# pierric/smart-chess-rust

Measured on AMD Instinct MI355X. Metric: MCTS simulations/sec (whole node), self-play rollout=180, at 1/2/4/8 MI355X, higher is better.
Workload: dtype bf16

## Files before the change

smart-chess-rust_amd/csrc/chess_history.hpp:

```cpp
#pragma once
#include "chess_rules.hpp"

namespace sc {

template <class Chain>
SC_HD bool is_repetition(const Chain& ch, int idx, int count) {
    bb_t key0 = ch.pos(idx).key;
    int i = idx;
    for (;;) {
        if (count <= 1) return true;
        if (i < count - 1) break;
        bool irrev = (ch.pos(i).flags & F_IRREV) != 0;
        i--;
        if (irrev) break;
        if (ch.pos(i).key == key0) count--;
    }
    return false;
}

enum { T_NONE = 0, T_CHECKMATE = 1, T_STALEMATE = 2, T_INSUFFICIENT = 3, T_SEVENTYFIVE = 4, T_FIVEFOLD = 5, T_FIFTY = 6, T_THREEFOLD = 7 };

template <class Chain>
SC_HD int outcome_claim_draw(const Chain& ch, int idx, int* winner) {
    const Position& p = ch.pos(idx);
    move_t buf1[MAX_MOVES], buf2[MAX_MOVES];
    MoveList l{buf1, 0};
    bool in_check = gen_legal(p, l);
    *winner = -1;
    if (in_check && l.n == 0) {
        *winner = !p.turn;
        return T_CHECKMATE;
    }
    if (insufficient_side(p, WHITE) && insufficient_side(p, BLACK)) return T_INSUFFICIENT;
    if (l.n == 0) return T_STALEMATE;
    if (p.halfmove >= 150) return T_SEVENTYFIVE;
    if (is_repetition(ch, idx, 5)) return T_FIVEFOLD;
    if (p.halfmove >= 100) return T_FIFTY;
    if (p.halfmove >= 99) {
        for (int i = 0; i < l.n; i++) {
            if (is_zeroing(p, l.m[i])) continue;
            Position q = p;
            make_move(q, l.m[i]);
            MoveList l2{buf2, 0};
            gen_legal(q, l2);
            if (q.halfmove >= 100 && l2.n > 0) return T_FIFTY;
        }
    }
    int lo = idx;
    while (lo > 0 && !(ch.pos(lo).flags & F_IRREV)) lo--;
    int cnt = 1;
    for (int i = lo; i < idx; i++)
        if (ch.pos(i).key == p.key) cnt++;
    if (cnt >= 3) return T_THREEFOLD;
    for (int j = 0; j < l.n; j++) {
        Position q = p;
        make_move(q, l.m[j]);
        int c2 = q.key == p.key ? 1 : 0;
        for (int i = lo; i < idx; i++)
            if (ch.pos(i).key == q.key) c2++;
        if (c2 >= 2) return T_THREEFOLD;
    }
    return T_NONE;
}

template <class Chain>
SC_HD void encode_cell(const Chain& ch, int idx, int px, int8_t* cell ) {
    int turn = ch.pos(idx).turn;
    int src = turn == BLACK ? (px ^ 56) : px;
    bb_t sb = bit(src);
    for (int j = 0; j < 8; j++) {
        int8_t* c = cell + 14 * j;
        for (int k = 0; k < 14; k++) c[k] = 0;
        if (j > idx) continue;
        const Position& h = ch.pos(idx - j);
        if ((h.occ[0] | h.occ[1]) & sb) {
            int t = piece_type_at(h, src);
            int is_white = (h.occ[WHITE] & sb) ? 1 : 0;
            int mover_side = turn == BLACK ? !is_white : is_white;
            c[t + (mover_side ? 0 : 6)] = 1;
        }
        c[12] = (h.flags & F_REP2) ? 1 : 0;
        c[13] = (h.flags & F_REP3) ? 1 : 0;
    }
}
SC_HD void encode_meta(const Position& p, int32_t* meta ) {
    int t = p.turn;
    uint8_t mk_ = t ? 1 : 4, mq = t ? 2 : 8, ok = t ? 4 : 1, oq = t ? 8 : 2;
    meta[0] = t;
    meta[1] = p.fullmove;
    meta[2] = (p.castling & mk_) != 0;
    meta[3] = (p.castling & mq) != 0;
    meta[4] = (p.castling & ok) != 0;
    meta[5] = (p.castling & oq) != 0;
    meta[6] = p.halfmove;
}

template <class Chain>
SC_HD uint8_t repetition_flags(const Chain& ch, int idx) {
    uint8_t f = 0;
    if (is_repetition(ch, idx, 2)) f |= F_REP2;
    if (is_repetition(ch, idx, 3)) f |= F_REP3;
    return f;
}

}
```

smart-chess-rust_amd/csrc/mcts_kernels.hip:

```cpp
#include "search_expand.hpp"

#include "launchers.hpp"

namespace sc {
__global__ __launch_bounds__(64) void k_debug_find_max(const float* u, int n, int* out) {
    const int lane = threadIdx.x;
    if (n <= 64) {
        const int r = wave_argmax_last_lane(lane < n ? u[lane] : 0.f, lane < n);
        if (lane == 0) out[0] = r;
    } else if (lane == 0) {
        out[0] = -2;
    }
    float best_u = 0.f;
    int best_i = -1;
#pragma unroll
    for (int r = 0; r < 4; r++) {
        const int i = lane + 64 * r;
        if (i < n) {
            const float v = u[i];
            if (best_i < 0 || v >= best_u) {
                best_u = v;
                best_i = i;
            }
        }
    }
    const int r4 = wave_argmax_last(best_u, best_i);
    if (lane == 0) out[1] = r4;
}

__global__ __launch_bounds__(64) void k_synth_eval(SpParams p) {
    const int g = blockIdx.x, lane = threadIdx.x;
    GameCtl& c = p.ctl[g];
    if (c.status != ST_ACTIVE || c.leaf_kind != LK_EVAL) return;
    const Position& pos = p.tpos[(size_t)g * p.tpos_cap + c.n_exp];
    uint64_t h = synth_pos_hash(pos) ^ p.synth_salt;
    int n = c.n_legal;
    const uint16_t* lm = p.legal_mv + (size_t)g * MAXC;
    if (p.evaluator == SYNTH_UNIFORM) {
        for (int i = lane; i < n; i += 64) p.prior[(size_t)g * MAXC + i] = 1.0f / (float)n;
        if (lane == 0) p.value[g] = 0.0f;
        return;
    }
    const bool coarse = p.evaluator == SYNTH_COARSE;
    unsigned long long sum = 0;
    for (int i = lane; i < n; i += 64) sum += coarse ? 1u + (synth_weight(h, lm[i]) >> 22) : synth_weight(h, lm[i]);
    sum = scw::wave_sum_u64(sum);
    float fs = (float)sum;
    for (int i = lane; i < n; i += 64)
        p.prior[(size_t)g * MAXC + i] = (float)(coarse ? 1u + (synth_weight(h, lm[i]) >> 22) : synth_weight(h, lm[i])) / fs;
    if (lane == 0) {
        const float v = synth_value(h);
        p.value[g] = coarse ? (v < -0.5f ? -0.5f : v >= 0.5f ? 0.5f : 0.0f) : v;
    }
}

__device__ inline int match_white(const SpParams& p, unsigned long long k) { return p.match_colours ? (int)(k & 1) : 0; }
__device__ inline unsigned long long match_ordinal(SpParams& p, int lane, int side) {
    const unsigned long long total = (unsigned long long)p.total_games;
    if (!p.match_colours && side) return total;
    unsigned long long n = 0;
    if (lane == 0) n = atomicAdd(&p.cnt->match_next[side], 1ULL);
    n = __shfl(n, 0, 64);
    const unsigned long long k = p.match_colours ? 2ULL * n + (unsigned long long)side : n;
    return k < total ? k : total;
}
__device__ inline int match_line_of(const SpParams& p, const MatchLines& ln, unsigned long long k) {
    return (int)((p.match_colours ? k >> 1 : k) % (unsigned long long)ln.n);
}
__device__ inline void match_copy_line(SpParams& p, int g, int lane, const Position* line, int len) {
    constexpr int W = (int)(sizeof(Position) / 8);
    static_assert(sizeof(Position) % 8 == 0, "a record is copied in 8-byte words");
    const unsigned long long* src = reinterpret_cast<const unsigned long long*>(line);
    unsigned long long* hist = reinterpret_cast<unsigned long long*>(p.hist + (size_t)g * p.hist_cap);
    unsigned long long* root = reinterpret_cast<unsigned long long*>(p.tpos + (size_t)g * p.tpos_cap);
    const int words = (len + 1) * W;
    wave_sync();
    for (int i = lane; i < words; i += 64) hist[i] = src[i];
    if (lane < W) root[lane] = src[len * W + lane];
    if (lane == 0) {
        p.ctl[g].ply = len;
        p.ctl[g].start_ply = len;
    }
}
__device__ inline void match_slot_start(SpParams& p, const MatchLines& ln, int g, int lane) {
    GameCtl& c = p.ctl[g];
    const int st = c.status, side = p.match_side & 1;
    const unsigned long long total = (unsigned long long)p.total_games;
    unsigned long long k;
    if (st == ST_MATCH_WAIT) {
        k = c.game_id - p.first_game_id;
    } else if (st == ST_IDLE) {
        k = match_ordinal(p, lane, side);
        if (k >= total) k = match_ordinal(p, lane, side ^ 1);
        if (k >= total) return;
    } else {
        return;
    }
    wave_sync();
    int len = 0;
    const Position* line = nullptr;
    if (ln.n > 0) {
        const int i = match_line_of(p, ln, k);
        const uint32_t a = ln.off[i], b = ln.off[i + 1];
        line = ln.tab + a;
        len = (int)(b - a) - 1;
    }
    if (side == (match_white(p, k) ^ (len & 1))) {
        try_start_game(p, g, lane, k);
        int now = 0;
        if (lane == 0) {
            now = c.status;
            if (now == ST_PENDING) c.status = ST_MATCH_WAIT;
        }
        if (len > 0 && __shfl(now, 0, 64) == ST_ACTIVE) match_copy_line(p, g, lane, line, len);
    } else if (lane == 0) {
        c.status = ST_MATCH_WAIT;
        c.leaf_kind = LK_NONE;
        c.game_id = p.first_game_id + k;
    }
}
__global__ __launch_bounds__(64) void k_match_boundary(SpParams p, MatchLines ln, int phase) {
    const int g = blockIdx.x, lane = threadIdx.x;
    if (phase == 1) {
        match_slot_start(p, ln, g, lane);
        return;
    }
    GameCtl& c = p.ctl[g];
    if (lane != 0 || c.status != ST_IDLE || c.trace_slot < 0) return;
    const TraceHdr& th = p.thdr[c.trace_slot];
    const int w = match_white(p, c.game_id - p.first_game_id);
    const int r = !th.has_outcome ? 3 : th.winner == 1 ? 0 : th.winner == 0 ? 1 : 2;
    p.match_tally()[((size_t)g * 2 + w) * 4 + r] += 1;
    c.trace_slot = -1;
}

__global__ __launch_bounds__(64) void k_init_slots(SpParams p, MatchLines ln) {
    const int g = blockIdx.x, lane = threadIdx.x;
    uint4* b = reinterpret_cast<uint4*>(p.boards + (size_t)g * 7168);
    for (int i = lane; i < 448; i += 64) b[i] = make_uint4(0, 0, 0, 0);
    if (lane < 8) p.meta[(size_t)g * 8 + lane] = 0;
    if (lane == 0) p.n_legal[g] = 0;
    if (p.match_recycle) {
        if (lane == 0) {
            p.ctl[g].status = ST_IDLE;
            p.ctl[g].leaf_kind = LK_NONE;
            p.ctl[g].trace_slot = -1;
        }
        wave_sync();
        match_slot_start(p, ln, g, lane);
        return;
    }
    if (g == 0 && lane == 0)
        atomicAdd(&p.cnt->next_game, (unsigned long long)(p.n_slots < p.total_games ? p.n_slots : p.total_games));
    if (g >= p.total_games) {
        if (lane == 0) {
            p.ctl[g].status = ST_IDLE;
            p.ctl[g].leaf_kind = LK_NONE;
        }
        return;
    }
    try_start_game(p, g, lane, (unsigned long long)g);
}

__global__ __launch_bounds__(64) void k_debug_choose_child(int n_cases, const int32_t* n_act, const int32_t* nc, const float* temperature,
                                                           const float* u, int tie_random, const float* w, const int32_t* w_off, int w_max,
                                                           int32_t* choice, float* total) {
    const int c = blockIdx.x, lane = threadIdx.x;
    if (c >= n_cases) return;
    float tot;
    const int ch = choose_child(n_act + (size_t)c * MAXC, uniform(nc[c]), temperature[c], u[c], tie_random, lane, w + uniform(w_off[c]), w_max, &tot);
    if (lane == 0) {
        choice[c] = ch;
        total[c] = tot;
    }
}

__global__ __launch_bounds__(64) void k_mcts(SpParams p, int do_expand, int do_select) {
    const int g = blockIdx.x, lane = threadIdx.x;
    __shared__ __attribute__((aligned(16))) int8_t s_stage[7168];
    __shared__ move_t s_moves[MAXC];
    __shared__ Position s_pos;
    __shared__ Position s_hist[8];
    __shared__ uint16_t s_ps[DEPTH_LDS];
    constexpr bool SC_ST = true;
    SC_STAMP(0);
    GameCtl cs_pre{};
    bool cs_pre_valid = false;
    if (do_expand) {
        dev_expand(p, g, lane, &s_pos, cs_pre, cs_pre_valid);
        __builtin_amdgcn_wave_barrier();
    }
    SC_STAMP(1);
    if (do_select) dev_select(p, g, lane, s_stage, s_moves, &s_pos, s_ps, s_hist, cs_pre, cs_pre_valid);
}

__global__ __launch_bounds__(64) void k_match_tally(const int32_t* tally, int n_slots, long long* out) {
    const int j = threadIdx.x;
    if (j >= 8) return;
    long long s = 0;
    for (int g = 0; g < n_slots; g++) s += tally[(size_t)g * 8 + j];
    out[j] = s;
}

__global__ __launch_bounds__(64) void k_open_lines(int n_lines, const uint16_t* moves, const uint32_t* move_off, Position* tab,
                                                   const uint32_t* rec_off, int32_t* status, Bases bases) {
    const int i = blockIdx.x, lane = threadIdx.x;
    if (i >= n_lines) return;
    __shared__ move_t s_moves[MAXC];
    __shared__ Position s_np;
    const uint16_t* mv = moves + move_off[i];
    const int nm = (int)(move_off[i + 1] - move_off[i]);
    const int pad = (int)(rec_off[i + 1] - rec_off[i]) - 1 - nm;
    Position* hist = tab + rec_off[i] + (pad > 0 ? pad : 0);
    Position cur = chain_start(bases, i, true);
    if (lane == 0) {
        Position none;
        set_startpos(none);
#pragma unroll
        for (int t = 0; t < 6; t++) none.pcs[t] = 0;
        none.occ[0] = none.occ[1] = 0;
        none.castling = 0;
        for (int k = 0; k < pad; k++) tab[rec_off[i] + k] = none;
        hist[0] = cur;
    }
    __syncthreads();
    int st = 0;
    for (int j = 0; j < nm; j++) {
        int nlm = 0;
        gen_legal_wave(cur, s_moves, lane, nlm);
        __syncthreads();
        bool found = false;
        for (int k = 0; k < nlm; k++)
            if (s_moves[k] == mv[j]) found = true;
        __syncthreads();
        if (!found) {
            st = -(j + 1);
            break;
        }
        replay_step(cur, mv[j], j, hist, hist, &s_np, lane);
    }
    if (st == 0) {
        int n = 0, winner = -1;
        gen_legal_wave(cur, s_moves, lane, n);
        __syncthreads();
        const HistChain hc{hist};
        if (outcome_claim_draw(hc, nm, &winner) != T_NONE || n == 0) st = 1;
    }
    if (lane == 0 && pad > 0) hist[0].flags = F_IRREV;
    if (lane == 0) status[i] = st;
}

__global__ __launch_bounds__(64) void k_set_position(SpParams p, int g, const uint16_t* moves, int n_moves, const Position* base) {
    const int lane = threadIdx.x;
    GameCtl& c = p.ctl[g];
    Position* hist = p.hist + (size_t)g * p.hist_cap;
    Position* tpos = p.tpos + (size_t)g * p.tpos_cap;
    __shared__ Position s_np;
    Position cur;
    if (base) {
        cur = uniform(*base);
    } else {
        set_startpos(cur);
        cur.key = position_key(cur);
    }
    if (lane == 0) hist[0] = cur;
    __syncthreads();
    for (int i = 0; i < n_moves && i + 1 < p.hist_cap; i++) replay_step(cur, moves[i], i, hist, tpos, &s_np, lane);
    if (lane == 0) {
        const size_t nb = (size_t)g * p.node_cap;
        tpos[0] = cur;
        p.N[nb] = 0;
        p.W[nb] = 0.0f;
        p.H[nb] = NodeHdr{-1, 0, 0};
        c.ply = n_moves;
        c.start_ply = n_moves;
        c.sim = 0;
        c.n_nodes = 1;
        c.n_exp = 1;
        c.leaf_kind = LK_NONE;
        c.rollout_cur = p.rollout;
        c.status = ST_ACTIVE;
    }
}

}

namespace scl {
void init_slots(const sc::SpParams& p, const sc::MatchLines& lines, hipStream_t s) {
    hipLaunchKernelGGL(sc::k_init_slots, dim3(p.n_slots), dim3(64), 0, s, p, lines);
}
void mcts(const sc::SpParams& p, int do_expand, int do_select, hipStream_t s) {
    hipLaunchKernelGGL(sc::k_mcts, dim3(p.n_slots), dim3(64), 0, s, p, do_expand, do_select);
}
void synth_eval(const sc::SpParams& p, hipStream_t s) { hipLaunchKernelGGL(sc::k_synth_eval, dim3(p.n_slots), dim3(64), 0, s, p); }
void debug_find_max(const float* d_u, int n, int* d_out, hipStream_t s) { hipLaunchKernelGGL(sc::k_debug_find_max, dim3(1), dim3(64), 0, s, d_u, n, d_out); }
void debug_choose_child(int n_cases, const int32_t* d_n_act, const int32_t* d_nc, const float* d_temperature, const float* d_u, int tie_random,
                        const float* d_w, const int32_t* d_w_off, int w_max, int32_t* d_choice, float* d_total, hipStream_t s) {
    if (n_cases <= 0) return;
    hipLaunchKernelGGL(sc::k_debug_choose_child, dim3(n_cases), dim3(64), 0, s, n_cases, d_n_act, d_nc, d_temperature, d_u, tie_random,
                       d_w, d_w_off, w_max, d_choice, d_total);
}
void match_boundary(const sc::SpParams& p, const sc::MatchLines& lines, hipStream_t s) {
    hipLaunchKernelGGL(sc::k_match_boundary, dim3(p.n_slots), dim3(64), 0, s, p, lines, 0);
    hipLaunchKernelGGL(sc::k_match_boundary, dim3(p.n_slots), dim3(64), 0, s, p, lines, 1);
}
void open_lines(int n_lines, const uint16_t* d_moves, const uint32_t* d_move_off, sc::Position* d_tab, const uint32_t* d_rec_off,
                int32_t* d_status, const sc::Bases& bases, hipStream_t s) {
    if (n_lines <= 0) return;
    hipLaunchKernelGGL(sc::k_open_lines, dim3(n_lines), dim3(64), 0, s, n_lines, d_moves, d_move_off, d_tab, d_rec_off, d_status, bases);
}
void match_tally(const int32_t* d_tally, int n_slots, long long* d_out, hipStream_t s) {
    hipLaunchKernelGGL(sc::k_match_tally, dim3(1), dim3(64), 0, s, d_tally, n_slots, d_out);
}
void set_position(const sc::SpParams& p, int slot, const uint16_t* d_moves, int n_moves, hipStream_t s, const sc::Position* d_base) {
    hipLaunchKernelGGL(sc::k_set_position, dim3(1), dim3(64), 0, s, p, slot, d_moves, n_moves, d_base);
}
}
```

smart-chess-rust_amd/csrc/position_chain.hpp:

```cpp
#pragma once
#include <hip/hip_runtime.h>

#include "chess_history.hpp"
#include "chess_rules_wave.hpp"
#include "encode_types.hpp"
#include "wave_util.hpp"

namespace sc {

using scw::uniform, scw::wave_sync;
__device__ __forceinline__ Position uniform(const Position& q) {
    Position r;
#pragma unroll
    for (int t = 0; t < 6; t++) r.pcs[t] = uniform(q.pcs[t]);
    r.occ[0] = uniform(q.occ[0]);
    r.occ[1] = uniform(q.occ[1]);
    r.key = uniform(q.key);
    r.turn = (uint8_t)uniform((int)q.turn);
    r.castling = (uint8_t)uniform((int)q.castling);
    r.ep = (int8_t)uniform((int)q.ep);
    r.flags = (uint8_t)uniform((int)q.flags);
    r.halfmove = (uint16_t)uniform((int)q.halfmove);
    r.fullmove = (uint16_t)uniform((int)q.fullmove);
    return r;
}

__device__ __forceinline__ Position chain_start(const Bases& b, int g, bool keyed) {
    Position cur;
    const int bi = b.rec ? uniform(b.idx[g]) : -1;
    if (bi >= 0) {
        cur = uniform(b.rec[bi]);
    } else {
        set_startpos(cur);
        if (keyed) cur.key = position_key(cur);
    }
    if (!keyed) cur.key = cur.flags = 0;
    return cur;
}

struct DevChain {
    const Position* hist;
    int root_ply;
    const Position* tpos;
    const uint16_t* ps_by_depth;
    const Position* leaf;
    int leaf_idx;
    __device__ const Position& pos(int i) const {
        if (i <= root_ply) return hist[i];
        if (i == leaf_idx) return *leaf;
        return tpos[ps_by_depth[i - root_ply]];
    }
};
struct HistChain {
    const Position* hist;
    __device__ const Position& pos(int i) const { return hist[i]; }
};

template <class Chain>
__device__ inline uint8_t rep_flags_wave(const Chain& ch, int idx, bb_t key0, int lane) {
    int matches = 0;
    for (int base = 0;; base += 64) {
        int i = idx - base - lane;
        bool valid = i >= 1;
        bool irrev = false, match = false;
        if (valid) {
            irrev = (ch.pos(i).flags & F_IRREV) != 0;
            match = ch.pos(i - 1).key == key0;
        }
        unsigned long long stopmask = __ballot(irrev || !valid);
        unsigned long long matchmask = __ballot(match && valid);
        bool stopped = stopmask != 0;
        if (stopped) {
            int first = __ffsll((long long)stopmask) - 1;
            matchmask &= first == 0 ? 0ULL : (~0ULL >> (64 - first));
        }
        matches += __popcll(matchmask);
        if (stopped || matches >= 2) break;
    }
    return (uint8_t)((matches >= 1 ? F_REP2 : 0) | (matches >= 2 ? F_REP3 : 0));
}

template <class Chain>
__device__ inline void stage_history(const Chain& ch, int idx, int lane, Position* s_hist) {
    const int j = lane >> 3, w = lane & 7;
    if (j <= idx) {
        const unsigned long long* src = reinterpret_cast<const unsigned long long*>(&ch.pos(idx - j));
        unsigned long long* dst = reinterpret_cast<unsigned long long*>(&s_hist[j]);
        dst[w] = src[w];
        if (w < 2) dst[8 + w] = src[8 + w];
    }
}

__device__ inline void encode_wave(const Position* s_hist, int n_hist, int lane, int8_t* stage, int8_t* out, int32_t* meta_out) {
    uint4* cell16 = reinterpret_cast<uint4*>(stage + lane * 112);
#pragma unroll
    for (int k = 0; k < 7; k++) cell16[k] = make_uint4(0, 0, 0, 0);
    int8_t* cell = stage + lane * 112;
    const int turn = s_hist[0].turn;
    int src = turn == BLACK ? (lane ^ 56) : lane;
    bb_t sb = bit(src);
    for (int j = 0; j < n_hist; j++) {
        const Position& h = s_hist[j];
        bb_t ow = h.occ[WHITE], ob = h.occ[BLACK];
        if ((ow | ob) & sb) {
            int t = 0;
#pragma unroll
            for (int k = 1; k < 6; k++)
                if (h.pcs[k] & sb) t = k;
            int is_white = (ow & sb) ? 1 : 0;
            int mover_side = turn == BLACK ? !is_white : is_white;
            cell[14 * j + t + (mover_side ? 0 : 6)] = 1;
        }
        uint8_t f = h.flags;
        cell[14 * j + 12] = (f & F_REP2) ? 1 : 0;
        cell[14 * j + 13] = (f & F_REP3) ? 1 : 0;
    }
    if (out) {
        uint4* o16 = reinterpret_cast<uint4*>(out + lane * 112);
#pragma unroll
        for (int k = 0; k < 7; k++) o16[k] = cell16[k];
    }
    if (lane == 0) {
        int32_t m[7];
        encode_meta(s_hist[0], m);
#pragma unroll
        for (int k = 0; k < 7; k++) meta_out[k] = m[k];
        meta_out[7] = 0;
    }
}

__device__ __forceinline__ void write_meta_row(const RowOut& o, int g, int lane) {
    if (!o.meta || lane >= 7) return;
    const int32_t* m = o.meta_s + (size_t)g * 7;
    int32_t v = m[lane];
    if (o.apply_mirror) v = lane == 0 ? 1 - m[0] : lane == 1 ? m[1] + (m[0] == 1 ? 1 : 0) : lane == 2 ? m[4] : lane == 3 ? m[5] : lane == 4 ? m[2] : lane == 5 ? m[3] : v;
    if (o.layout == 1) static_cast<float*>(o.meta)[(size_t)g * 7 + lane] = (float)v;
    else static_cast<int32_t*>(o.meta)[(size_t)g * 7 + lane] = v;
}

__device__ inline bb_t position_key_wave(const Position& p, int lane, bool ep_legal) {
    bb_t h = 0;
    if ((all_occ(p) >> lane) & 1) h = psq_key(piece_type_at(p, lane), (int)((p.occ[WHITE] >> lane) & 1), lane);
    unsigned lo = (unsigned)h, hi = (unsigned)(h >> 32);
    for (int o = 32; o > 0; o >>= 1) {
        lo ^= (unsigned)__shfl_xor((int)lo, o, 64);
        hi ^= (unsigned)__shfl_xor((int)hi, o, 64);
    }
    return (((bb_t)hi << 32) | lo) ^ state_key(p.turn, p.castling, ep_legal ? p.ep : -1);
}

__device__ inline void replay_step(Position& cur, move_t m, int i, Position* hist, const Position* tpos, Position* s_np, int lane) {
    make_move(cur, m);
    if (lane == 0) *s_np = cur;
    __syncthreads();
    DevChain ch{hist, i, tpos, nullptr, s_np, i + 1};
    uint8_t rf = rep_flags_wave(ch, i + 1, cur.key, lane);
    cur.flags = (uint8_t)((cur.flags & F_IRREV) | rf);
    __syncthreads();
    if (lane == 0) hist[i + 1] = cur;
    __threadfence_block();
    __syncthreads();
}

}
```

smart-chess-rust_amd/csrc/rules_host_api.cpp:

```cpp
#include <stdlib.h>
#include <string.h>
#include <vector>

#include "chess_history.hpp"

using namespace sc;

struct sct_state {
    std::vector<Position> hist;
    std::vector<move_t> moves;
    const Position& pos(int i) const { return hist[(size_t)i]; }
};

static void finalize_rep(sct_state* s) {
    int idx = (int)s->hist.size() - 1;
    s->hist[(size_t)idx].flags |= repetition_flags(*s, idx);
}

extern "C" {

sct_state* sct_new() {
    sct_state* s = new sct_state();
    Position p;
    set_startpos(p);
    p.key = position_key(p);
    s->hist.push_back(p);
    return s;
}
void sct_free(sct_state* s) { delete s; }
void sct_reset(sct_state* s) {
    Position p;
    set_startpos(p);
    p.key = position_key(p);
    s->hist.assign(1, p);
    s->moves.clear();
}
int sct_set_fen(sct_state* s, const char* fen) {
    Position p;
    memset(&p, 0, sizeof p);
    int r = 7, f = 0;
    const char* c = fen;
    const char* names = "pnbrqk";
    for (; *c && *c != ' '; c++) {
        if (*c == '/') { r--; f = 0; continue; }
        if (*c >= '1' && *c <= '8') { f += *c - '0'; continue; }
        bool white = *c >= 'A' && *c <= 'Z';
        char lc = (char)(white ? *c + 32 : *c);
        const char* q = strchr(names, lc);
        if (!q || r < 0 || f > 7) return -1;
        int sq = r * 8 + f;
        p.pcs[q - names] |= bit(sq);
        p.occ[white ? WHITE : BLACK] |= bit(sq);
        f++;
    }
    if (*c != ' ') return -1;
    c++;
    p.turn = *c == 'w';
    c++;
    while (*c == ' ') c++;
    for (; *c && *c != ' '; c++) {
        if (*c == 'K') p.castling |= 1;
        if (*c == 'Q') p.castling |= 2;
        if (*c == 'k') p.castling |= 4;
        if (*c == 'q') p.castling |= 8;
    }
    bb_t wk = p.pcs[KING] & p.occ[WHITE], bk = p.pcs[KING] & p.occ[BLACK];
    bb_t wr = p.pcs[ROOK] & p.occ[WHITE], br = p.pcs[ROOK] & p.occ[BLACK];
    if (!(wk & bit(4))) p.castling &= (uint8_t)~3;
    if (!(bk & bit(60))) p.castling &= (uint8_t)~12;
    if (!(wr & bit(7))) p.castling &= (uint8_t)~1;
    if (!(wr & bit(0))) p.castling &= (uint8_t)~2;
    if (!(br & bit(63))) p.castling &= (uint8_t)~4;
    if (!(br & bit(56))) p.castling &= (uint8_t)~8;
    while (*c == ' ') c++;
    p.ep = -1;
    if (*c && *c != '-') {
        p.ep = (int8_t)((c[1] - '1') * 8 + (c[0] - 'a'));
        c += 2;
    } else if (*c)
        c++;
    p.halfmove = 0;
    p.fullmove = 1;
    while (*c == ' ') c++;
    if (*c) {
        p.halfmove = (uint16_t)strtol(c, (char**)&c, 10);
        while (*c == ' ') c++;
        if (*c) p.fullmove = (uint16_t)strtol(c, NULL, 10);
    }
    p.key = position_key(p);
    s->hist.assign(1, p);
    s->moves.clear();
    return 0;
}
int sct_turn(const sct_state* s) { return s->hist.back().turn; }
void sct_get_fields(const sct_state* s, uint64_t* out ) {
    const Position& p = s->hist.back();
    for (int t = 0; t < 6; t++) out[t] = p.pcs[t];
    out[6] = p.occ[0];
    out[7] = p.occ[1];
    out[8] = p.turn;
    out[9] = p.castling;
    out[10] = (uint64_t)(int64_t)p.ep;
    out[11] = p.halfmove;
    out[12] = p.fullmove;
}
void sct_push(sct_state* s, uint16_t m) {
    Position p = s->hist.back();
    make_move(p, m);
    s->hist.push_back(p);
    s->moves.push_back(m);
    finalize_rep(s);
}
void sct_pop(sct_state* s) {
    s->hist.pop_back();
    s->moves.pop_back();
}
int sct_legal_moves(const sct_state* s, uint16_t* out, int* in_check) {
    move_t buf[MAX_MOVES];
    MoveList l{buf, 0};
    bool chk = gen_legal(s->hist.back(), l);
    if (in_check) *in_check = chk;
    memcpy(out, l.m, sizeof(move_t) * (size_t)l.n);
    return l.n;
}
static uint64_t perft(const Position& p, int depth) {
    move_t buf[MAX_MOVES];
    MoveList l{buf, 0};
    gen_legal(p, l);
    if (depth == 1) return (uint64_t)l.n;
    uint64_t t = 0;
    for (int i = 0; i < l.n; i++) {
        Position q = p;
        make_move(q, l.m[i]);
        t += perft(q, depth - 1);
    }
    return t;
}
uint64_t sct_perft(const sct_state* s, int depth) { return depth <= 0 ? 1 : perft(s->hist.back(), depth); }
int sct_is_repetition(const sct_state* s, int count) { return is_repetition(*s, (int)s->hist.size() - 1, count); }
int sct_outcome(const sct_state* s, int* winner) { return outcome_claim_draw(*s, (int)s->hist.size() - 1, winner); }
void sct_encode(const sct_state* s, int8_t* boards, int32_t* meta) {
    int idx = (int)s->hist.size() - 1;
    for (int px = 0; px < 64; px++) encode_cell(*s, idx, px, boards + px * 112);
    encode_meta(s->hist.back(), meta);
}
int sct_move_index(uint16_t m, int turn) { return move_index(m, turn); }
uint64_t sct_pos_hash(const sct_state* s) { return synth_pos_hash(s->hist.back()); }
uint64_t sct_key(const sct_state* s) { return s->hist.back().key; }
uint64_t sct_key_full(const sct_state* s) { return position_key(s->hist.back()); }
uint64_t sct_rng(uint64_t a, uint64_t b, uint64_t c, uint64_t d, uint64_t e) { return sc_rng(a, b, c, d, e); }
int sct_board_diff_legal(const sct_state* s, int* n_moves) {
    move_t buf[MAX_MOVES];
    MoveList l{buf, 0};
    const Position& p = s->hist.back();
    gen_legal(p, l);
    int diff = 0;
    for (int i = 0; i < l.n; i++) {
        Position a = p, b = p;
        make_move(a, l.m[i]);
        make_move_board(b, l.m[i]);
        if (memcmp(a.pcs, b.pcs, sizeof a.pcs)) diff |= 1;
        if (memcmp(a.occ, b.occ, sizeof a.occ)) diff |= 2;
        if (a.castling != b.castling) diff |= 4;
        if (a.ep != b.ep) diff |= 8;
        if (a.halfmove != b.halfmove) diff |= 16;
        if (a.fullmove != b.fullmove) diff |= 32;
        if (a.turn != b.turn) diff |= 64;
    }
    if (n_moves) *n_moves = l.n;
    return diff;
}
void sct_synth_eval(const sct_state* s, float* priors, float* value) {
    move_t buf[MAX_MOVES];
    MoveList l{buf, 0};
    gen_legal(s->hist.back(), l);
    uint64_t h = synth_pos_hash(s->hist.back());
    uint64_t sum = 0;
    for (int i = 0; i < l.n; i++) sum += synth_weight(h, l.m[i]);
    for (int i = 0; i < l.n; i++) priors[i] = (float)synth_weight(h, l.m[i]) / (float)sum;
    *value = synth_value(h);
}
}
```

smart-chess-rust_amd/csrc/search_expand.hpp:

```cpp
#pragma once
#include "search_select.hpp"
#include "value_tail.hpp"

namespace sc {
__device__ inline void try_start_game(SpParams& p, int g, int lane, unsigned long long k) {
    GameCtl& c = p.ctl[g];
    const int ts = (int)(k % (unsigned long long)p.trace_cap);
    const int st = p.thdr[ts].state;
    const unsigned long long prev_id = p.thdr[ts].game_id;
    bool ok;
    if (k < (unsigned long long)p.trace_cap) ok = st == TR_FREE;
    else ok = prev_id == p.first_game_id + k - (unsigned long long)p.trace_cap && (st == TR_FREE || (st == TR_DONE && !p.trace_hold));
    if (!ok) {
        if (lane == 0) {
            c.status = ST_PENDING;
            c.leaf_kind = LK_NONE;
            c.game_id = p.first_game_id + k;
        }
        return;
    }
    const size_t nb = (size_t)g * p.node_cap;
    if (lane == 0) {
        Position s;
        set_startpos(s);
        s.key = position_key(s);
        p.hist[(size_t)g * p.hist_cap] = s;
        p.tpos[(size_t)g * p.tpos_cap] = s;
        p.N[nb] = 0;
        p.W[nb] = 0.0f;
        p.P[nb] = 0.0f;
        p.U[nb] = 0.0f;
        p.MV[nb] = 0;
        p.H[nb] = NodeHdr{-1, 0, 0};
        c.status = ST_ACTIVE;
        c.ply = 0;
        c.start_ply = 0;
        c.sim = 0;
        c.n_nodes = 1;
        c.n_exp = 1;
        c.leaf = 0;
        c.path_len = 0;
        c.leaf_kind = LK_NONE;
        c.n_legal = 0;
        c.err = 0;
        c.rollout_cur = p.rollout;
        c.game_id = p.first_game_id + k;
        c.trace_slot = ts;
        TraceHdr& th = p.thdr[ts];
        th.n_steps = 0;
        th.has_outcome = 0;
        th.termination = 0;
        th.winner = -1;
        th.game_id = c.game_id;
        th.state = TR_LIVE;
    }
}
__device__ inline void start_new_game(SpParams& p, int g, int lane) {
    GameCtl& c = p.ctl[g];
    unsigned long long k = 0;
    if (lane == 0) k = atomicAdd(&p.cnt->next_game, 1ULL);
    k = __shfl(k, 0, 64);
    if (k >= (unsigned long long)p.total_games) {
        if (lane == 0) {
            c.status = ST_IDLE;
            c.leaf_kind = LK_NONE;
        }
        return;
    }
    try_start_game(p, g, lane, k);
}

__device__ inline void finish_game(SpParams& p, int g, int lane, int has_outcome, int term, int winner) {
    GameCtl& c = p.ctl[g];
    if (lane == 0) {
        TraceHdr& th = p.thdr[c.trace_slot];
        th.n_steps = c.ply - c.start_ply;
        th.has_outcome = has_outcome;
        th.termination = term;
        th.winner = winner;
        th.game_id = c.game_id;
        __threadfence();
        th.state = TR_DONE;
        atomicAdd(&p.cnt->games_finished, 1);
        c.status = ST_FINISHED;
    }
    wave_sync();
    start_new_game(p, g, lane);
}

__device__ inline int choose_child(const int32_t* n_act, int nc, float temperature, float u, int tie_random, int lane, const float* w,
                                   int w_max, float* total) {
    *total = 0.0f;
    if (temperature == 0.0f) {
        int bn = -1, bi = 0x7fffffff;
        for (int i = lane; i < nc; i += 64) {
            int n = n_act[i];
            if (n > bn) {
                bn = n;
                bi = i;
            }
        }
        for (int o = 32; o > 0; o >>= 1) {
            int on = __shfl_xor(bn, o, 64), oi = __shfl_xor(bi, o, 64);
            if (on > bn || (on == bn && oi < bi)) {
                bn = on;
                bi = oi;
            }
        }
        int choice = bi;
        if (tie_random) {
            int cnt = 0;
            for (int i = 0; i < nc; i++) cnt += n_act[i] == bn;
            int k = (int)(u * (float)cnt);
            if (k >= cnt) k = cnt - 1;
            for (int i = 0; i < nc; i++)
                if (n_act[i] == bn && k-- == 0) {
                    choice = i;
                    break;
                }
        }
        return choice;
    }
    const bool plain = 1.0f / temperature == 1.0f;
    auto weight = [&](int n) { return plain ? (float)n : w[n < w_max ? n : w_max]; };
    float sum = 0.0f;
    for (int i = 0; i < nc; i++) sum += weight(n_act[i]);
    *total = sum;
    float x = u * sum;
    float cum = 0.0f;
    int idx = 0;
    for (int i = 0; i < nc - 1; i++) {
        cum += weight(n_act[i]);
        if (cum <= x) idx++;
    }
    return idx;
}

using scvt::ValueTail;
__device__ __forceinline__ void value_tail_issue(const SpParams& p, int g, int lane, ValueTail& t) {
    const float* wf = p.vf_w;
    const int32_t* meta = p.meta + (size_t)g * 8;
#pragma unroll
    for (int k = 0; k < 7; k++) t.meta[k] = meta[k];
    const int j = 2 * lane;
    const float* vp = p.vpart + (size_t)g * 128 + j;
    const size_t vstride = (size_t)p.n_slots * 128;
#pragma unroll
    for (int ks = 0; ks < 32; ks++) t.acc[ks] = *reinterpret_cast<const float2*>(vp + (size_t)ks * vstride);
    if (p.vf_ksplit > 32) {
#pragma unroll
        for (int ks = 32; ks < 64; ks++) t.acc[ks] = *reinterpret_cast<const float2*>(vp + (size_t)ks * vstride);
    } else {
#pragma unroll
        for (int ks = 32; ks < 64; ks++) t.acc[ks] = make_float2(0.f, 0.f);
    }
    t.bias = *reinterpret_cast<const float2*>(wf + p.vf_fc1b + j);
    t.w2 = *reinterpret_cast<const float2*>(wf + p.vf_fc2w + j);
#pragma unroll
    for (int k = 0; k < 7; k++) t.wm[k] = *reinterpret_cast<const float2*>(wf + p.vf_fc1m + k * 128 + j);
    t.fc2b = wf[p.vf_fc2b];
}
__device__ __forceinline__ float value_tail_finish(const SpParams& p, const ValueTail& t) { return scvt::value_tail_compute(t, p.vf_ksplit); }

template <bool SC_ST = true>
__device__ __forceinline__ void dev_expand(SpParams& p, int g, int lane, Position* s_np_p, GameCtl& cs_out, bool& cs_valid) {
#pragma clang fp contract(off)
    Position& s_np = *s_np_p;
    GameCtl& c = p.ctl[g];
    {
        const void *a0 = p.ctl, *a1 = p.path, *a2 = p.prior, *a3 = p.legal_mv, *a4 = p.slot_cnt, *a5 = p.vpart, *a6 = p.vf_w, *a7 = p.meta;
        const int i0 = p.max_depth, i1 = p.vf_fused, i2 = p.n_slots, i3 = p.vf_ksplit;
        const uint32_t u0 = p.vf_fc1b, u1 = p.vf_fc1m, u2 = p.vf_fc2w, u3 = p.vf_fc2b;
        asm volatile("" ::"s"(a0), "s"(a1), "s"(a2), "s"(a3), "s"(a4), "s"(a5), "s"(a6), "s"(a7), "s"(i0), "s"(i1), "s"(i2), "s"(i3), "s"(u0), "s"(u1),
                     "s"(u2), "s"(u3));
    }
    const GameCtl craw = c;
    const int pth_raw = p.path[(size_t)g * p.max_depth + (lane < p.max_depth ? lane : p.max_depth - 1)];
    float prv[4];
    uint16_t lmv[4];
#pragma unroll
    for (int k = 0; k < 4; k++) {
        const int i = lane + 64 * k, ic = i < MAXC ? i : MAXC - 1;
        prv[k] = p.prior[(size_t)g * MAXC + ic];
        lmv[k] = p.legal_mv[(size_t)g * MAXC + ic];
    }
    const unsigned long long sc_sims = p.slot_cnt[(size_t)g * 2], sc_evals = p.slot_cnt[(size_t)g * 2 + 1];
    ValueTail vt;
    if (p.vf_fused) value_tail_issue(p, g, lane, vt);
    __builtin_amdgcn_sched_barrier(0);
    SC_XSTAMP(16);
    const GameCtl cs = uniform(craw);
    SC_XSTAMP(17);
    const int pth = lane < p.max_depth ? pth_raw : 0;
#pragma unroll
    for (int k = 0; k < 4; k++) {
        const int i = lane + 64 * k;
        prv[k] = i < MAXC ? prv[k] : 0.f;
        lmv[k] = i < MAXC ? lmv[k] : (uint16_t)0;
    }
    cs_out = cs;
    cs_valid = true;
    if (cs.status == ST_PENDING) {
        try_start_game(p, g, lane, cs.game_id - p.first_game_id);
        cs_valid = false;
        return;
    }
    if (cs.status != ST_ACTIVE || cs.leaf_kind == LK_NONE) return;
    const size_t nb = (size_t)g * p.node_cap;
    int32_t* N = p.N + nb;
    float* W = p.W + nb;
    float* P = p.P + nb;
    float* U = p.U + nb;
    uint16_t* MV = p.MV + nb;
    NodeHdr* H = p.H + nb;
    const int32_t* path = p.path + (size_t)g * p.max_depth;
    Position* hist = p.hist + (size_t)g * p.hist_cap;
    Position* tpos = p.tpos + (size_t)g * p.tpos_cap;

    const int leaf = cs.leaf, kind = cs.leaf_kind, plen = cs.path_len;
    float value = cs.leaf_value;
    int n_nodes = cs.n_nodes, n_exp = cs.n_exp;
    uint32_t err = 0;
    const bool inpath = lane < plen;
    int n0 = 0;
    float w0 = 0.f;
    if (inpath) {
        n0 = N[pth];
        w0 = W[pth];
    }
    if (kind == LK_EVAL) {
        value = p.vf_fused ? value_tail_finish(p, vt) : p.value[g];
        SC_XSTAMP(18);
        int n = cs.n_legal;
        if (n_nodes + n > p.node_cap || n_exp + 1 >= p.tpos_cap) {
            err = ERR_POOL_OVERFLOW;
        } else {
#pragma unroll
            for (int k = 0; k < 4; k++) {
                int i = lane + 64 * k;
                if (i < n) {
                    int id = n_nodes + i;
                    N[id] = 0;
                    W[id] = 0.0f;
                    P[id] = prv[k];
                    U[id] = 0.0f;
                    MV[id] = lmv[k];
                    H[id] = NodeHdr{-1, 0, 0};
                }
            }
            if (lane == 0) H[leaf] = NodeHdr{n_nodes, (uint16_t)n, (uint16_t)n_exp};
            n_nodes += n;
            n_exp += 1;
        }
    } else if (kind == LK_TERM_NEW) {
        if (lane == 0) H[leaf] = NodeHdr{value == 0.0f ? -2 : value > 0.0f ? -3 : -4, 0, 0};
    }
    SC_XSTAMP(19);
    if (inpath) {
        N[pth] = n0 + 1;
        W[pth] = w0 + value;
    }
    for (int d = lane + 64; d < plen; d += 64) {
        int nd = path[d];
        N[nd] += 1;
        W[nd] += value;
    }
    wave_sync();
    int sim = cs.sim + 1;
    if (lane == 0) {
        c.n_nodes = n_nodes;
        c.n_exp = n_exp;
        c.sim = sim;
        c.leaf_kind = LK_NONE;
        if (err) {
            c.err = cs.err | err;
            atomicOr(&p.cnt->err, (int)err);
        }
        p.slot_cnt[(size_t)g * 2] = sc_sims + 1ULL;
        if (kind == LK_EVAL) p.slot_cnt[(size_t)g * 2 + 1] = sc_evals + 1ULL;
    }
    SC_XSTAMP(20);
    cs_out.n_nodes = n_nodes;
    cs_out.n_exp = n_exp;
    cs_out.sim = sim;
    cs_out.leaf_kind = LK_NONE;
    cs_out.err = cs.err | err;
    const int budget = p.rollout_factor > 0.f ? cs.rollout_cur : p.rollout;
    if (sim < budget) return;
    cs_valid = false;

    wave_sync();
    const int ply = cs.ply;
    const NodeHdr h0 = H[0];
    const int nc = h0.nc, fc = h0.fc;
    if (nc == 0 || budget == 0) {
        HistChain hc{hist};
        int winner = -1;
        int term = outcome_claim_draw(hc, ply, &winner);
        finish_game(p, g, lane, term != T_NONE, term, winner);
        return;
    }
    const int ts = cs.trace_slot;
    const size_t tstep = (size_t)ts * p.num_steps + (size_t)(ply - cs.start_ply);
    for (int i = lane; i < nc; i += 64) {
        p.t_cmove[tstep * MAXC + i] = MV[fc + i];
        p.t_cn[tstep * MAXC + i] = N[fc + i];
        p.t_cq[tstep * MAXC + i] = W[fc + i];
        p.t_cu[tstep * MAXC + i] = U[fc + i];
    }
    const float temperature = (ply - cs.start_ply) < p.temp_switch ? 1.0f : p.temperature;
    const float u = (float)(sc_rng(p.seed, cs.game_id, (uint64_t)ply, 1, 0) >> 40) / 16777216.0f;
    float w_total;
    const int choice = choose_child(N + fc, nc, temperature, u, p.tie_random, lane, p.choice_w, p.choice_w_max, &w_total);
    move_t mv = MV[fc + choice];
    if (lane == 0) {
        p.t_move[tstep] = mv;
        p.t_q[tstep] = W[0];
        p.t_nchild[tstep] = nc;
    }
    Position np = uniform(hist[ply]);
    make_move(np, (move_t)uniform((int)mv));
    if (lane == 0) s_np = np;
    wave_sync();
    {
        DevChain ch{hist, ply, tpos, nullptr, &s_np, ply + 1};
        uint8_t rf = rep_flags_wave(ch, ply + 1, np.key, lane);
        np.flags = (uint8_t)((np.flags & F_IRREV) | rf);
    }
    wave_sync();
    if (lane == 0) {
        hist[ply + 1] = np;
        atomicAdd(&p.cnt->plies_done, 1ULL);
    }
    wave_sync();
    const int new_ply = ply + 1;
    if (lane == 0) c.ply = new_ply;
    const int i_step = ply - cs.start_ply;
    if (i_step > p.outcome_gate) {
        HistChain hc{hist};
        int winner = -1;
        int term = outcome_claim_draw(hc, new_ply, &winner);
        if (term != T_NONE) {
            wave_sync();
            finish_game(p, g, lane, 1, term, winner);
            return;
        }
    }
    if (i_step + 1 >= p.num_steps || new_ply + 1 >= p.hist_cap) {
        wave_sync();
        finish_game(p, g, lane, 0, 0, -1);
        return;
    }
    if (lane == 0) {
        tpos[0] = np;
        N[0] = 0;
        W[0] = 0.0f;
        P[0] = 0.0f;
        U[0] = 0.0f;
        MV[0] = mv;
        H[0] = NodeHdr{-1, 0, 0};
        c.n_nodes = 1;
        c.n_exp = 1;
        c.sim = 0;
    }
}

}
```

smart-chess-rust_amd/csrc/step_kernels.hip:

```cpp
#include "search_expand.hpp"
#include "nn_kernels.hpp"
#include "nn_tower32.hpp"

#include "launchers.hpp"
#include "tower_config.hpp"

namespace scstep {

__device__ __forceinline__ void fc1_tail(const scnn::TowerArgs& A, const sc::SpParams& p, const int g, const bool ran, scnn::Fc1Hand& fh) {
    const int tid = threadIdx.x, lane = tid & 63;
    const int wave = __builtin_amdgcn_readfirstlane(tid >> 6);
    const int mb = g >> 6, ks = g & 63;
    uint32_t* ctr = A.fc1_arrive + mb * 32;
#ifdef SC_EXP
#define TSTAMP(k) do { if (p.dbg_cycles && tid == 0) p.dbg_cycles[(size_t)g * 32 + 8 + (k)] = __builtin_amdgcn_s_memrealtime(); } while (0)
#else
#define TSTAMP(k)
#endif
    TSTAMP(0);
    if (!ran) {
        if (tid == 0) __hip_atomic_fetch_add(ctr, 1u, __ATOMIC_RELAXED, __HIP_MEMORY_SCOPE_AGENT);
        scnn::fc1_wload(fh.w, A.net, ks, 64, wave, lane);
        __builtin_amdgcn_sched_barrier(0);
    }
    const scnn::Fc1W& w = fh.w;
    const bool have_a = ran && fh.have_a;
#ifdef SC_EXP
    if (p.dbg_cycles && tid == 0) p.dbg_cycles[(size_t)g * 32 + 14] = have_a;
    if (have_a) { TSTAMP(1); TSTAMP(2); }
#endif
    if (tid == 0 && !have_a) {
        const uint64_t t0 = __builtin_amdgcn_s_memrealtime();
        uint32_t seen = ran ? fh.early : __hip_atomic_load(ctr, __ATOMIC_RELAXED, __HIP_MEMORY_SCOPE_AGENT);
        while ((int32_t)(seen - A.fc1_target) < 0) {
            __builtin_amdgcn_s_sleep(4);
            const uint64_t waited = __builtin_amdgcn_s_memrealtime() - t0;
            if (waited > 20000000ull) {
                atomicOr(&p.cnt->err, sc::ERR_HANDOFF_TIMEOUT);
                break;
            }
            if (waited > 100000ull && (__hip_atomic_load(&p.cnt->err, __ATOMIC_RELAXED, __HIP_MEMORY_SCOPE_AGENT) & sc::ERR_HANDOFF_TIMEOUT)) break;
            seen = __hip_atomic_load(ctr, __ATOMIC_RELAXED, __HIP_MEMORY_SCOPE_AGENT);
        }
        TSTAMP(1);
        if (A.fc1_acquire) __builtin_amdgcn_fence(__ATOMIC_ACQUIRE, "agent");
        asm volatile("s_waitcnt vmcnt(0)" ::: "memory");
        TSTAMP(2);
    }
    __syncthreads();
    scnn::bf16_t* s_a = reinterpret_cast<scnn::bf16_t*>(scnn::g_smem);
    if (!have_a) scnn::fc1_load_a(fh.a, A.hval, mb, ks, tid);
    scnn::fc1_put_a(s_a, fh.a, tid);
    __syncthreads();
    TSTAMP(3);
    scnn::fc1_mma_store(w, s_a, A.vpart, A.n_pos, mb, ks, 64, wave, lane);
    TSTAMP(4);
#ifdef SC_EXP
    asm volatile("s_waitcnt vmcnt(0)" ::: "memory");
    TSTAMP(5);
#endif
}

template <class P, int C, int RS, int TPI, int AB, bool STAMPS = false>
__global__ __launch_bounds__(256, 1) void k_step(scnn::TowerArgs A, sc::SpParams p, int do_expand) {
    __shared__ __attribute__((aligned(16))) int8_t s_stage[7168];
    __shared__ sc::move_t s_moves[sc::MAXC];
    __shared__ sc::Position s_pos;
    __shared__ sc::Position s_hist[8];
    __shared__ uint16_t s_ps[sc::DEPTH_LDS];
    __shared__ sc::HelperBox s_box;
    const int g = blockIdx.x;
    const int lane = threadIdx.x & 63;
#ifdef SC_EXP
    const long long t_entry = clock64();
#endif
    scnn::kernarg_prefetch<sizeof(scnn::TowerArgs) + sizeof(sc::SpParams) + sizeof(int)>();
#ifdef SC_EXP
    if (p.dbg_cycles && threadIdx.x == 0) p.dbg_cycles[(size_t)g * 32 + 21] = t_entry;
#endif
#define PHASE_STAMP(k, cond) do { if constexpr (STAMPS) { if (p.dbg_cycles && (cond)) p.dbg_cycles[(size_t)g * 32 + (k)] = __builtin_amdgcn_s_memrealtime(); } } while (0)
    PHASE_STAMP(24, threadIdx.x == 0);
    if (threadIdx.x == 0) s_box.state = 0;
    __syncthreads();
    auto search = [&](int wave) -> bool {
        if (wave == 1) {
            sc::dev_encode_helper(p, g, lane, &s_box, s_stage, &s_pos, s_ps, s_hist);
            return true;
        }
        constexpr bool SC_ST = STAMPS || SC_ST_DEFAULT;
        SC_STAMP(0);
        sc::GameCtl cs_pre{};
        bool cs_pre_valid = false;
        if (do_expand) {
            sc::dev_expand<SC_ST>(p, g, lane, &s_pos, cs_pre, cs_pre_valid);
            __builtin_amdgcn_wave_barrier();
        }
        SC_STAMP(1);
        const bool need_net = sc::dev_select<false, SC_ST>(p, g, lane, s_stage, s_moves, &s_pos, s_ps, s_hist, cs_pre, cs_pre_valid, &s_box);
        PHASE_STAMP(25, lane == 0);
        return need_net;
    };
    scnn::Fc1Hand fh;
    const bool ran = scnn::tower_body<P, C, RS, TPI, AB>(A, g, s_stage, search, fh);
    PHASE_STAMP(26, threadIdx.x == 0);
    if (A.fc1_arrive) fc1_tail(A, p, g, ran, fh);
    PHASE_STAMP(27, threadIdx.x == 0);
#undef PHASE_STAMP
}

}

namespace scl {
#define K_STEP(P, C, RS, TPI, AB) scstep::k_step<scnn::P, C, RS, TPI, AB>
#define K_STEP_STAMPED scstep::k_step<scnn::PrecBF16, 128, SC_T32_RS, SC_T32_TPI, SC_T32_AB, true>
const char* step_init() {
    const void* kn[4] = {reinterpret_cast<const void*>(&K_STEP(PrecBF16, 128, SC_T32_RS, SC_T32_TPI, SC_T32_AB)),
                         reinterpret_cast<const void*>(&K_STEP(PrecBF16, 256, SC_T32W_RS, SC_T32W_TPI, SC_T32W_AB)),
                         reinterpret_cast<const void*>(&K_STEP(PrecFP8, 128, SC_T8_RS, SC_T8_TPI, SC_T8_AB)),
                         reinterpret_cast<const void*>(&K_STEP(PrecFP8, 256, SC_T8W_RS, SC_T8W_TPI, SC_T8W_AB))};
    for (int i = 0; i < 4; i++) {
        hipError_t e = hipFuncSetAttribute(kn[i], hipFuncAttributeMaxDynamicSharedMemorySize, scnn::tower32_lds_bytes(i & 1 ? 256 : 128, i >= 2 && i < 4));
        if (e != hipSuccess) return hipGetErrorString(e);
    }
    {
        hipError_t e = hipFuncSetAttribute(reinterpret_cast<const void*>(&K_STEP_STAMPED), hipFuncAttributeMaxDynamicSharedMemorySize, scnn::tower32_lds_bytes(128));
        if (e != hipSuccess) return hipGetErrorString(e);
    }
    return nullptr;
}
int step_blocks_per_cu(const scnn::NetLayout& net) {
    int n = 0;
    hipError_t e;
    if (net.fp8 && net.C == 128)
        e = hipOccupancyMaxActiveBlocksPerMultiprocessor(&n, K_STEP(PrecFP8, 128, SC_T8_RS, SC_T8_TPI, SC_T8_AB), 256, scnn::tower32_lds_bytes(128, true));
    else if (net.fp8)
        e = hipOccupancyMaxActiveBlocksPerMultiprocessor(&n, K_STEP(PrecFP8, 256, SC_T8W_RS, SC_T8W_TPI, SC_T8W_AB), 256, scnn::tower32_lds_bytes(256, true));
    else if (net.C == 128)
        e = hipOccupancyMaxActiveBlocksPerMultiprocessor(&n, K_STEP(PrecBF16, 128, SC_T32_RS, SC_T32_TPI, SC_T32_AB), 256, scnn::tower32_lds_bytes(128));
    else
        e = hipOccupancyMaxActiveBlocksPerMultiprocessor(&n, K_STEP(PrecBF16, 256, SC_T32W_RS, SC_T32W_TPI, SC_T32W_AB), 256, scnn::tower32_lds_bytes(256));
    return e == hipSuccess && n > 0 ? n : 1;
}
void step(const scnn::TowerArgs& a, const sc::SpParams& p, int do_expand, hipStream_t s) {
    const dim3 grid(p.n_slots), block(256);
    if (a.net.fp8 && a.net.C == 128)
        hipLaunchKernelGGL((K_STEP(PrecFP8, 128, SC_T8_RS, SC_T8_TPI, SC_T8_AB)), grid, block, scnn::tower32_lds_bytes(128, true), s, a, p, do_expand);
    else if (a.net.fp8)
        hipLaunchKernelGGL((K_STEP(PrecFP8, 256, SC_T8W_RS, SC_T8W_TPI, SC_T8W_AB)), grid, block, scnn::tower32_lds_bytes(256, true), s, a, p, do_expand);
    else if (a.net.C == 128 && p.dbg_cycles)
        hipLaunchKernelGGL((K_STEP_STAMPED), grid, block, scnn::tower32_lds_bytes(128), s, a, p, do_expand);
    else if (a.net.C == 128)
        hipLaunchKernelGGL((K_STEP(PrecBF16, 128, SC_T32_RS, SC_T32_TPI, SC_T32_AB)), grid, block, scnn::tower32_lds_bytes(128), s, a, p, do_expand);
    else
        hipLaunchKernelGGL((K_STEP(PrecBF16, 256, SC_T32W_RS, SC_T32W_TPI, SC_T32W_AB)), grid, block, scnn::tower32_lds_bytes(256), s, a, p, do_expand);
}
}
```

Measured before the change: 2.209 million.

## Parallelize game-outcome draw detection across wave lanes

Adds a lane-generic outcome_claim_draw_lanes that uses wave-parallel legal move generation into shared memory and ballots for the repetition scans and the per-move threefold claim checks. dev_expand now calls it in place of the serial per-thread outcome check, with a compile-time switch and a host mirror kept for testing. The aim is to stop every lane redundantly running the whole serial move generation and history scans at each expansion. It adds wave syncs and regenerates moves inside the fifty-move loop, and the fivefold test is folded into a single count, which could differ subtly from the original logic.

```diff
diff --git a/smart-chess-rust_amd/csrc/chess_history.hpp b/smart-chess-rust_amd/csrc/chess_history.hpp
--- a/smart-chess-rust_amd/csrc/chess_history.hpp
+++ b/smart-chess-rust_amd/csrc/chess_history.hpp
@@ -63,6 +63,63 @@
     return T_NONE;
 }
 
+template <class Lanes, class Chain>
+SC_HD int outcome_claim_draw_lanes(Lanes& w, const Chain& ch, int idx, int* winner) {
+    const Position p = w.uniform(ch.pos(idx));
+    int n = 0;
+    const bool in_check = w.gen_legal(p, n);
+    *winner = -1;
+    if (in_check && n == 0) {
+        *winner = !p.turn;
+        return T_CHECKMATE;
+    }
+    if (insufficient_side(p, WHITE) && insufficient_side(p, BLACK)) return T_INSUFFICIENT;
+    if (n == 0) return T_STALEMATE;
+    if (p.halfmove >= 150) return T_SEVENTYFIVE;
+    int lo = 0;
+    for (int base = 0;; base += 64) {
+        const unsigned long long stop = w.ballot([&](int l) {
+            const int i = idx - base - l;
+            return i <= 0 || (ch.pos(i).flags & F_IRREV) != 0;
+        });
+        if (stop) {
+            lo = idx - base - __builtin_ctzll(stop);
+            break;
+        }
+    }
+    int cnt = 0;
+    for (int base = lo; base < idx; base += 64)
+        cnt += __builtin_popcountll(w.ballot([&](int l) { return base + l < idx && ch.pos(base + l).key == p.key; }));
+    if (cnt >= 4) return T_FIVEFOLD;
+    if (p.halfmove >= 100) return T_FIFTY;
+    if (p.halfmove >= 99) {
+        for (int i = 0; i < n; i++) {
+            const move_t m = w.moves[i];
+            if (is_zeroing(p, m)) continue;
+            Position q = p;
+            make_move(q, m);
+            int n2 = 0;
+            w.gen_legal(q, n2);
+            if (q.halfmove >= 100 && n2 > 0) return T_FIFTY;
+            w.gen_legal(p, n);
+        }
+    }
+    if (cnt >= 2) return T_THREEFOLD;
+    for (int base = 0; base < n; base += 64) {
+        const unsigned long long claim = w.ballot([&](int l) {
+            if (base + l >= n) return false;
+            Position q = p;
+            make_move(q, w.moves[base + l]);
+            int c2 = q.key == p.key ? 1 : 0;
+            for (int i = lo; i < idx; i++)
+                if (ch.pos(i).key == q.key) c2++;
+            return c2 >= 2;
+        });
+        if (claim) return T_THREEFOLD;
+    }
+    return T_NONE;
+}
+
 template <class Chain>
 SC_HD void encode_cell(const Chain& ch, int idx, int px, int8_t* cell ) {
     int turn = ch.pos(idx).turn;
diff --git a/smart-chess-rust_amd/csrc/mcts_kernels.hip b/smart-chess-rust_amd/csrc/mcts_kernels.hip
--- a/smart-chess-rust_amd/csrc/mcts_kernels.hip
+++ b/smart-chess-rust_amd/csrc/mcts_kernels.hip
@@ -187,7 +187,7 @@
     GameCtl cs_pre{};
     bool cs_pre_valid = false;
     if (do_expand) {
-        dev_expand(p, g, lane, &s_pos, cs_pre, cs_pre_valid);
+        dev_expand(p, g, lane, &s_pos, s_moves, cs_pre, cs_pre_valid);
         __builtin_amdgcn_wave_barrier();
     }
     SC_STAMP(1);
diff --git a/smart-chess-rust_amd/csrc/position_chain.hpp b/smart-chess-rust_amd/csrc/position_chain.hpp
--- a/smart-chess-rust_amd/csrc/position_chain.hpp
+++ b/smart-chess-rust_amd/csrc/position_chain.hpp
@@ -54,6 +54,24 @@
 struct HistChain {
     const Position* hist;
     __device__ const Position& pos(int i) const { return hist[i]; }
+};
+
+struct WaveLanes {
+    move_t* moves;
+    int lane;
+    __device__ Position uniform(const Position& q) const { return sc::uniform(q); }
+    __device__ bool gen_legal(const Position& p, int& n) {
+        wave_sync();
+        int nn = 0;
+        const bool chk = gen_legal_wave(p, moves, lane, nn);
+        wave_sync();
+        n = scw::uniform(nn);
+        return chk;
+    }
+    template <class F>
+    __device__ unsigned long long ballot(F f) const {
+        return __ballot(f(lane));
+    }
 };
 
 template <class Chain>
diff --git a/smart-chess-rust_amd/csrc/rules_host_api.cpp b/smart-chess-rust_amd/csrc/rules_host_api.cpp
--- a/smart-chess-rust_amd/csrc/rules_host_api.cpp
+++ b/smart-chess-rust_amd/csrc/rules_host_api.cpp
@@ -10,6 +10,24 @@
     std::vector<Position> hist;
     std::vector<move_t> moves;
     const Position& pos(int i) const { return hist[(size_t)i]; }
+};
+
+struct HostLanes {
+    move_t buf[MAX_MOVES];
+    move_t* moves = buf;
+    Position uniform(const Position& q) const { return q; }
+    bool gen_legal(const Position& p, int& n) {
+        MoveList l{buf, 0};
+        const bool chk = sc::gen_legal(p, l);
+        n = l.n;
+        return chk;
+    }
+    template <class F>
+    unsigned long long ballot(F f) const {
+        unsigned long long m = 0;
+        for (int l = 0; l < 64; l++) m |= (unsigned long long)(f(l) ? 1 : 0) << l;
+        return m;
+    }
 };
 
 static void finalize_rep(sct_state* s) {
@@ -139,6 +157,10 @@
 uint64_t sct_perft(const sct_state* s, int depth) { return depth <= 0 ? 1 : perft(s->hist.back(), depth); }
 int sct_is_repetition(const sct_state* s, int count) { return is_repetition(*s, (int)s->hist.size() - 1, count); }
 int sct_outcome(const sct_state* s, int* winner) { return outcome_claim_draw(*s, (int)s->hist.size() - 1, winner); }
+int sct_outcome_lanes(const sct_state* s, int* winner) {
+    HostLanes w;
+    return outcome_claim_draw_lanes(w, *s, (int)s->hist.size() - 1, winner);
+}
 void sct_encode(const sct_state* s, int8_t* boards, int32_t* meta) {
     int idx = (int)s->hist.size() - 1;
     for (int px = 0; px < 64; px++) encode_cell(*s, idx, px, boards + px * 112);
diff --git a/smart-chess-rust_amd/csrc/search_expand.hpp b/smart-chess-rust_amd/csrc/search_expand.hpp
--- a/smart-chess-rust_amd/csrc/search_expand.hpp
+++ b/smart-chess-rust_amd/csrc/search_expand.hpp
@@ -162,8 +162,21 @@
 }
 __device__ __forceinline__ float value_tail_finish(const SpParams& p, const ValueTail& t) { return scvt::value_tail_compute(t, p.vf_ksplit); }
 
+#ifndef SC_CLAIM_DRAW_WAVE
+#define SC_CLAIM_DRAW_WAVE 1
+#endif
+template <class Chain>
+__device__ __forceinline__ int dev_outcome(const Chain& ch, int idx, int* winner, move_t* s_moves, int lane) {
+#if SC_CLAIM_DRAW_WAVE
+    WaveLanes w{s_moves, lane};
+    return outcome_claim_draw_lanes(w, ch, idx, winner);
+#else
+    return outcome_claim_draw(ch, idx, winner);
+#endif
+}
+
 template <bool SC_ST = true>
-__device__ __forceinline__ void dev_expand(SpParams& p, int g, int lane, Position* s_np_p, GameCtl& cs_out, bool& cs_valid) {
+__device__ __forceinline__ void dev_expand(SpParams& p, int g, int lane, Position* s_np_p, move_t* s_moves, GameCtl& cs_out, bool& cs_valid) {
 #pragma clang fp contract(off)
     Position& s_np = *s_np_p;
     GameCtl& c = p.ctl[g];
@@ -296,7 +309,7 @@
     if (nc == 0 || budget == 0) {
         HistChain hc{hist};
         int winner = -1;
-        int term = outcome_claim_draw(hc, ply, &winner);
+        int term = dev_outcome(hc, ply, &winner, s_moves, lane);
         finish_game(p, g, lane, term != T_NONE, term, winner);
         return;
     }
@@ -339,7 +352,7 @@
     if (i_step > p.outcome_gate) {
         HistChain hc{hist};
         int winner = -1;
-        int term = outcome_claim_draw(hc, new_ply, &winner);
+        int term = dev_outcome(hc, new_ply, &winner, s_moves, lane);
         if (term != T_NONE) {
             wave_sync();
             finish_game(p, g, lane, 1, term, winner);
diff --git a/smart-chess-rust_amd/csrc/step_kernels.hip b/smart-chess-rust_amd/csrc/step_kernels.hip
--- a/smart-chess-rust_amd/csrc/step_kernels.hip
+++ b/smart-chess-rust_amd/csrc/step_kernels.hip
@@ -92,7 +92,7 @@
         sc::GameCtl cs_pre{};
         bool cs_pre_valid = false;
         if (do_expand) {
-            sc::dev_expand<SC_ST>(p, g, lane, &s_pos, cs_pre, cs_pre_valid);
+            sc::dev_expand<SC_ST>(p, g, lane, &s_pos, s_moves, cs_pre, cs_pre_valid);
             __builtin_amdgcn_wave_barrier();
         }
         SC_STAMP(1);
```

New measurement: 2.207 million. About the same (-0.1%).
